# ucuapps/OpenGlue

Hardware: NVIDIA H100
Metric: image-pairs/sec at N=M=2048, d=256, 9 GNN layers, 100 Sinkhorn iters (higher is better)
Workload: dtype fp16x3 (fp16 hi/lo operands with power-of-two tensor scales, 3 products, fp32 accumulate)

## Files before the change

openglue_b200/csrc/sinkhorn.cuh:

```cuda
#pragma once
#include "common.cuh"
#include "tc_common.cuh"
#include <math_constants.h>
#include <algorithm>

namespace og {

struct SinkArgs {
  static constexpr bool kBackward = false;
  const float* S; int64_t lds, strideS;
  const float* dustbin;
  int B, n, m, iters;
  float reg;
  float norm, log_a_last, log_b_last;
  float* scores;
  float* u;
  float* partial;
  unsigned int* barrier;
  int SP, rows_per_strip, mpad;
  int rows_smem;
  float* vglob;
  float* hist_u;
  float* hist_v;
};

constexpr int SINK_WARPS = 8;
constexpr int64_t SINK_BARRIER_BYTES = 256 * 128;
constexpr int SINK_MAX_COLS = 8192;
constexpr int SINK_MAX_STRIPS = 32;
constexpr float LOG2E_F = 1.4426950408889634f;

__device__ __forceinline__ void grid_barrier(unsigned int* counter, unsigned int target) {
  __syncthreads();
  if (threadIdx.x == 0) {
    __threadfence();
    atomicAdd(counter, 1u);
    unsigned int seen;
    do {
      asm volatile("ld.acquire.gpu.global.u32 %0, [%1];" : "=r"(seen) : "l"(counter) : "memory");
    } while (seen < target);
    __threadfence();
  }
  __syncthreads();
}

typedef unsigned long long f32x2;
__device__ __forceinline__ f32x2 pk2(float x, float y) { f32x2 r; asm("mov.b64 %0, {%1, %2};" : "=l"(r) : "f"(x), "f"(y)); return r; }
__device__ __forceinline__ void upk2(f32x2 v, float& x, float& y) { asm("mov.b64 {%0, %1}, %2;" : "=f"(x), "=f"(y) : "l"(v)); }
#define OG_F32X2_OP(name, expr)                                        \
  __device__ __forceinline__ f32x2 name(f32x2 a, f32x2 b) {            \
    float ax, ay, bx, by; upk2(a, ax, ay); upk2(b, bx, by);            \
    auto op = [](float u, float v) { return expr; };                   \
    return pk2(op(ax, bx), op(ay, by));                                \
  }
OG_F32X2_OP(add2, __fadd_rn(u, v))
OG_F32X2_OP(sub2, __fsub_rn(u, v))
OG_F32X2_OP(mul2, __fmul_rn(u, v))
#undef OG_F32X2_OP
__device__ __forceinline__ f32x2 fma2(f32x2 a, f32x2 b, f32x2 c) {
  float ax, ay, bx, by, cx, cy; upk2(a, ax, ay); upk2(b, bx, by); upk2(c, cx, cy);
  return pk2(__fmaf_rn(ax, bx, cx), __fmaf_rn(ay, by, cy));
}

template <int V, int W>
struct SinkStrip {
  static constexpr int C = 128 * V, MC = W * C, G = SINK_WARPS / W;
  int b, strip, tid, lane, grp, sub, c0, r0, r1;
  template <class Args>
  __device__ __forceinline__ explicit SinkStrip(const Args& a) {
    b = blockIdx.x / a.SP; strip = blockIdx.x % a.SP;
    tid = threadIdx.x; lane = tid & 31;
    grp = (tid >> 5) / W; sub = (tid >> 5) % W;
    c0 = sub * C;
    r0 = strip * a.rows_per_strip;
    r1 = min(r0 + a.rows_per_strip, a.n + 1);
  }
};

template <int V, int W, int SLOTS, bool EVICT_FIRST, class Args>
struct SinkRowRing {
  static constexpr int C = 128 * V, G = SINK_WARPS / W;
  float* slot;
  uint64_t* bar;
  const Args& a;
  const float* seg;
  int first, end_real, c0, lane;
  uint32_t bytes, consumed;
  bool full;
  float dz;
  uint64_t policy;

  __device__ __forceinline__ SinkRowRing(const Args& args, const SinkStrip<V, W>& s, float* ring, uint64_t* bars) : a(args) {
    const int warp = s.grp * W + s.sub;
    slot = ring + warp * SLOTS * C;
    bar = bars + warp * SLOTS;
    seg = a.S + (int64_t)s.b * a.strideS + s.c0;
    first = s.r0 + s.grp;
    end_real = min(s.r1, a.n);
    c0 = s.c0; lane = s.lane;
    const int seg_cols = min(a.m, c0 + C) - c0;
    bytes = seg_cols > 0 ? (uint32_t)(((seg_cols + 3) / 4) * 16) : 0u;
    full = seg_cols == C;
    consumed = 0;
    dz = (a.reg == 1.0f) ? __ldg(a.dustbin) : __fdiv_rn(__ldg(a.dustbin), a.reg);
    if (lane == 0) {
      for (int sl = 0; sl < SLOTS; ++sl) tc::mbar_init(&bar[sl], 1);
      tc::fence_barrier_init();
    }
    if (EVICT_FIRST) asm volatile("createpolicy.fractional.L2::evict_first.b64 %0, 1.0;" : "=l"(policy));
  }

  __device__ __forceinline__ void copy(uint32_t sl, int row) {
    tc::mbar_arrive_expect_tx(&bar[sl], bytes);
    const float* src = seg + (int64_t)row * a.lds;
    if (EVICT_FIRST)
      asm volatile("cp.async.bulk.shared::cluster.global.mbarrier::complete_tx::bytes.L2::cache_hint [%0], [%1], %2, [%3], %4;"
                   ::"r"(tc::smem_u32(slot + sl * C)), "l"(src), "r"(bytes), "r"(tc::smem_u32(&bar[sl])), "l"(policy) : "memory");
    else
      asm volatile("cp.async.bulk.shared::cluster.global.mbarrier::complete_tx::bytes [%0], [%1], %2, [%3];"
                   ::"r"(tc::smem_u32(slot + sl * C)), "l"(src), "r"(bytes), "r"(tc::smem_u32(&bar[sl])) : "memory");
  }

  __device__ __forceinline__ void prime() {
    if (lane == 0 && bytes) {
      for (int sl = 0; sl < SLOTS; ++sl) {
        const int row = first + sl * G;
        if (row < end_real) copy((consumed + sl) % SLOTS, row);
      }
    }
  }

  __device__ __forceinline__ void take(int row, float4 (&z)[V]) {
    if (row >= a.n) {
#pragma unroll
      for (int k = 0; k < V; ++k) z[k] = make_float4(dz, dz, dz, dz);
      return;
    }
    if (!bytes) {
#pragma unroll
      for (int k = 0; k < V; ++k) z[k] = make_float4(0.f, 0.f, 0.f, 0.f);
      return;
    }
    const uint32_t sl = consumed % SLOTS, ph = (consumed / SLOTS) & 1;
    while (!tc::mbar_try_wait(&bar[sl], ph)) {}
    const float4* src = reinterpret_cast<const float4*>(slot + sl * C);
    if (full) {
#pragma unroll
      for (int k = 0; k < V; ++k) z[k] = src[lane + 32 * k];
    } else {
#pragma unroll
      for (int k = 0; k < V; ++k) {
        const int idx = lane + 32 * k;
        const int c = c0 + 4 * idx;
        const int m = a.m;
        float4 q = (c < m) ? src[idx] : make_float4(0.f, 0.f, 0.f, 0.f);
        if (c < m && c + 3 >= m) {
          if (c + 1 >= m) q.y = 0.f;
          if (c + 2 >= m) q.z = 0.f;
          q.w = 0.f;
        }
        z[k] = q;
      }
    }
    ++consumed;
    __syncwarp();
    const int nxt = row + SLOTS * G;
    if (lane == 0 && nxt < end_real) copy(sl, nxt);
    if (a.reg != 1.0f) {
      const float reg = a.reg;
#pragma unroll
      for (int k = 0; k < V; ++k) {
        z[k].x = __fdiv_rn(z[k].x, reg); z[k].y = __fdiv_rn(z[k].y, reg);
        z[k].z = __fdiv_rn(z[k].z, reg); z[k].w = __fdiv_rn(z[k].w, reg);
      }
    }
  }
};

template <int V, int W, class X>
__device__ __forceinline__ const X* sink_row_exchange(X* xr, X mine, const SinkStrip<V, W>& s, uint32_t& rowpar) {
  X* x = xr + (rowpar * SinkStrip<V, W>::G + s.grp) * W;
  if (s.lane == 0) x[s.sub] = mine;
  asm volatile("bar.sync %0, %1;" ::"r"(1 + s.grp), "n"(W * 32) : "memory");
  rowpar ^= 1u;
  return x;
}

template <int V, int W, class Args, class Store>
__device__ __forceinline__ void sink_strip_sums(const Args& a, const SinkStrip<V, W>& s, float* red, const float4 (&cacc)[V],
                                                float cacc_m, Store store) {
  const int m = a.m;
  float* myred = red + s.grp * a.mpad;
#pragma unroll
  for (int q = 0; q < V; ++q) {
    const int c = s.c0 + 4 * (s.lane + 32 * q);
    if (c < m) *reinterpret_cast<float4*>(myred + c) = cacc[q];
  }
  __syncthreads();
  if (s.sub == 0 && s.lane == 0) myred[m] = cacc_m;
  __syncthreads();
  for (int j = s.tid; j <= m; j += blockDim.x) {
    float sum = 0.f;
#pragma unroll
    for (int w = 0; w < SinkStrip<V, W>::G; ++w) sum += red[w * a.mpad + j];
    store(j, sum);
  }
}

template <int V, int W, class Args, class Update>
__device__ __forceinline__ void sink_column_reduce(const Args& a, const SinkStrip<V, W>& s, float* red, const float4 (&cacc)[V],
                                                   float cacc_m, int k, Update update) {
  const int m = a.m;
  const int64_t buf = (int64_t)(k & 1) * a.B * a.SP + (int64_t)s.b * a.SP;
  float* part = a.partial + (buf + s.strip) * a.mpad;
  sink_strip_sums(a, s, red, cacc, cacc_m, [&](int j, float sum) { part[j] = sum; });
  grid_barrier(a.barrier + 32 * s.b, (unsigned int)(k + 1) * (unsigned int)a.SP);
  const float* pb = a.partial + buf * a.mpad;
  for (int j4 = s.tid; 4 * j4 <= m; j4 += blockDim.x) {
    float4 c = make_float4(0.f, 0.f, 0.f, 0.f);
#pragma unroll 8
    for (int sp = 0; sp < a.SP; ++sp) {
      const float4 q = __ldcg(reinterpret_cast<const float4*>(pb + (int64_t)sp * a.mpad) + j4);
      c.x += q.x; c.y += q.y; c.z += q.z; c.w += q.w;
    }
    const float cc[4] = {c.x, c.y, c.z, c.w};
#pragma unroll
    for (int e = 0; e < 4; ++e) {
      const int j = 4 * j4 + e;
      if (j < m) update(j, cc[e]);
      else if (j == m) update(SinkStrip<V, W>::MC, cc[e]);
    }
  }
  __syncthreads();
}

template <int V, int W>
__device__ __forceinline__ void sink_fwd_row(const SinkArgs& a, const SinkStrip<V, W>& s, const float4 (&q)[V], const float* v_s,
                                             float v_m, float dz, float a_reg, float a_last, float2* xr, uint32_t& rowpar, int row,
                                             int it, f32x2 (&cacc)[2 * V], float& cacc_m) {
  const int n = a.n, c0 = s.c0, lane = s.lane, sub = s.sub;
  const f32x2 log2e2 = pk2(LOG2E_F, LOG2E_F);
  f32x2 z[2 * V];
#pragma unroll
  for (int k = 0; k < V; ++k) { z[2 * k] = pk2(q[k].x, q[k].y); z[2 * k + 1] = pk2(q[k].z, q[k].w); }
  const float t_m = dz + v_m;
  float mx = (sub == 0) ? t_m : -CUDART_INF_F;
#pragma unroll
  for (int k = 0; k < V; ++k) {
    const ulonglong2 vv = *reinterpret_cast<const ulonglong2*>(v_s + c0 + 4 * (lane + 32 * k));
    z[2 * k] = add2(z[2 * k], vv.x); z[2 * k + 1] = add2(z[2 * k + 1], vv.y);
    float x0, x1, x2, x3; upk2(z[2 * k], x0, x1); upk2(z[2 * k + 1], x2, x3);
    mx = fmaxf(mx, fmaxf(fmaxf(x0, x1), fmaxf(x2, x3)));
  }
  mx = warp_max(mx);
  const float mxs = (mx == -CUDART_INF_F) ? 0.f : mx;
  const f32x2 mxs2 = pk2(mxs, mxs);
  f32x2 sum2a = 0ull, sum2b = 0ull;
#pragma unroll
  for (int k = 0; k < 2 * V; ++k) {
    float x, y; upk2(mul2(sub2(z[k], mxs2), log2e2), x, y);
    z[k] = pk2(ex2_approx(x), ex2_approx(y));
    if (k & 1) sum2b = add2(sum2b, z[k]); else sum2a = add2(sum2a, z[k]);
  }
  float sa, sb; upk2(add2(sum2a, sum2b), sa, sb);
  const float e_m = (sub == 0) ? ex2_approx((t_m - mxs) * LOG2E_F) : 0.f;
  float s_i = warp_sum(sa + sb) + e_m;
  float mxg = mx, f_w = 1.f;
  if (W > 1) {
    const float2* x = sink_row_exchange(xr, make_float2(mx, s_i), s, rowpar);
    float2 p[W];
#pragma unroll
    for (int w2 = 0; w2 < W; ++w2) { p[w2] = x[w2]; mxg = fmaxf(mxg, p[w2].x); }
    s_i = 0.f;
#pragma unroll
    for (int w2 = 0; w2 < W; ++w2) s_i = fmaf(p[w2].y, ex2_approx((p[w2].x - mxg) * LOG2E_F), s_i);
    f_w = ex2_approx((mx - mxg) * LOG2E_F);
  }
  const float w_i = __fdiv_rn((row < n) ? a_reg : a_last, s_i) * f_w;
  if ((it == a.iters - 1 || a.hist_u) && sub == 0 && lane == 0) {
    const float u_i = ((row < n) ? a.norm : a.log_a_last) - (mxg + logf(s_i));
    if (it == a.iters - 1) a.u[(int64_t)s.b * (n + 1) + row] = u_i;
    if (a.hist_u) a.hist_u[((int64_t)s.b * a.iters + it) * (n + 1) + row] = u_i;
  }
  const f32x2 w2 = pk2(w_i, w_i);
#pragma unroll
  for (int k = 0; k < 2 * V; ++k) cacc[k] = fma2(z[k], w2, cacc[k]);
  cacc_m = fmaf(e_m, w_i, cacc_m);
}

template <int V, int W>
__device__ __forceinline__ void sink_fwd_score_row(const SinkArgs& a, const SinkStrip<V, W>& s, const float4 (&z)[V], const float* v_s,
                                                   float v_m, float dz, int row) {
  const int n = a.n, m = a.m, c0 = s.c0, lane = s.lane;
  float u_i = 0.f;
  if (a.iters > 0) {
    if (lane == 0) u_i = __ldcg(a.u + (int64_t)s.b * (n + 1) + row);
    u_i = __shfl_sync(0xffffffffu, u_i, 0);
  }
  float* out = a.scores + ((int64_t)s.b * (n + 1) + row) * (m + 1);
#pragma unroll
  for (int k = 0; k < V; ++k) {
    const int c = c0 + 4 * (lane + 32 * k);
    if (c < m) {
      const float4 vv = *reinterpret_cast<const float4*>(v_s + c);
      if (c + 0 < m) out[c + 0] = (z[k].x + u_i) + vv.x - a.norm;
      if (c + 1 < m) out[c + 1] = (z[k].y + u_i) + vv.y - a.norm;
      if (c + 2 < m) out[c + 2] = (z[k].z + u_i) + vv.z - a.norm;
      if (c + 3 < m) out[c + 3] = (z[k].w + u_i) + vv.w - a.norm;
    }
  }
  if (s.sub == 0 && lane == 0) out[m] = (dz + u_i) + v_m - a.norm;
}

template <int V, int W, int SLOTS>
__global__ void __launch_bounds__(SINK_WARPS * 32, (V <= 8) ? 2 : 1) sinkhorn_kernel(SinkArgs a) {
  extern __shared__ __align__(128) float og_sink_smem[];
  using Strip = SinkStrip<V, W>;
  constexpr int C = Strip::C, MC = Strip::MC, G = Strip::G;
  float* v_s = og_sink_smem;
  float* red = og_sink_smem + MC + 4;
  float* ring = red + G * a.mpad;
  uint64_t* bars = reinterpret_cast<uint64_t*>(ring + SINK_WARPS * SLOTS * C);
  float2* xr = reinterpret_cast<float2*>(bars + SINK_WARPS * SLOTS);
  const Strip s(a);
  const int m = a.m;
  const float a_reg = expf(a.norm), a_last = expf(a.log_a_last);
  SinkRowRing<V, W, SLOTS, true, SinkArgs> rows(a, s, ring, bars);
  const float dz = rows.dz;

  for (int j = s.tid; j < MC; j += blockDim.x) v_s[j] = (j < m) ? 0.f : -CUDART_INF_F;
  if (s.tid == 0) v_s[MC] = 0.f;
  __syncthreads();

  rows.prime();
  uint32_t rowpar = 0;
  for (int it = 0; it < a.iters; ++it) {
    f32x2 cacc[2 * V];
#pragma unroll
    for (int k = 0; k < 2 * V; ++k) cacc[k] = 0ull;
    float cacc_m = 0.f;
    const float v_m = v_s[MC];

    for (int row = s.r0 + s.grp; row < s.r1; row += G) {
      float4 q[V];
      rows.take(row, q);
      sink_fwd_row(a, s, q, v_s, v_m, dz, a_reg, a_last, xr, rowpar, row, it, cacc, cacc_m);
    }
    rows.prime();
    float4 c4[V];
#pragma unroll
    for (int k = 0; k < V; ++k) { upk2(cacc[2 * k], c4[k].x, c4[k].y); upk2(cacc[2 * k + 1], c4[k].z, c4[k].w); }
    sink_column_reduce(a, s, red, c4, cacc_m, it, [&](int j, float c) {
      v_s[j] = ((j < MC) ? a.norm : a.log_b_last) + v_s[j] - logf(c);
    });
    if (a.hist_v && s.strip == 0) {
      float* hv = a.hist_v + ((int64_t)s.b * (a.iters + 1) + it + 1) * (m + 1);
      for (int j = s.tid; j <= m; j += blockDim.x) hv[j] = (j < m) ? v_s[j] : v_s[MC];
    }
  }

  const float v_m = v_s[MC];
  for (int row = s.r0 + s.grp; row < s.r1; row += G) {
    float4 z[V];
    rows.take(row, z);
    sink_fwd_score_row(a, s, z, v_s, v_m, dz, row);
  }
}

__device__ __forceinline__ void sink_put(uint64_t* p, float x, uint32_t tag) {
  asm volatile("st.relaxed.gpu.global.b64 [%0], %1;" ::"l"(p), "l"(((uint64_t)tag << 32) | __float_as_uint(x)) : "memory");
}
__device__ __forceinline__ uint64_t sink_get(const uint64_t* p) {
  uint64_t w;
  asm volatile("ld.relaxed.gpu.global.b64 %0, [%1];" : "=l"(w) : "l"(p) : "memory");
  return w;
}
constexpr int SINK_POLL = 16;
template <int N, class At>
__device__ __forceinline__ void sink_take(float (&x)[N], At at, uint32_t tag) {
  uint64_t w[N];
#pragma unroll
  for (int u = 0; u < N; ++u) { const uint64_t* p = at(u); w[u] = p ? sink_get(p) : (uint64_t)tag << 32; }
  for (;;) {
    bool ready = true;
#pragma unroll
    for (int u = 0; u < N; ++u) ready &= (uint32_t)(w[u] >> 32) == tag;
    if (ready) break;
#pragma unroll
    for (int u = 0; u < N; ++u)
      if ((uint32_t)(w[u] >> 32) != tag) w[u] = sink_get(at(u));
  }
#pragma unroll
  for (int u = 0; u < N; ++u) x[u] = __uint_as_float((uint32_t)w[u]);
}

template <int V, int W, int RR>
__global__ void __launch_bounds__(SINK_WARPS * 32, 1) sinkhorn_resident_kernel(SinkArgs a) {
  extern __shared__ __align__(128) float og_sink_smem[];
  using Strip = SinkStrip<V, W>;
  constexpr int C = Strip::C, MC = Strip::MC, G = Strip::G, NT = SINK_WARPS * 32;
  float* v_s = og_sink_smem;
  float* red = v_s + MC + 4;
  float* ring = red;
  float* gsum = red + max(G * a.mpad, SINK_WARPS * C);
  float4* held = reinterpret_cast<float4*>(gsum + NT);
  uint64_t* bars = reinterpret_cast<uint64_t*>(held + (size_t)SINK_WARPS * a.rows_smem * (C / 4));
  float2* xr = reinterpret_cast<float2*>(bars + SINK_WARPS);
  const Strip s(a);
  const int m = a.m, lane = s.lane;
  const float a_reg = expf(a.norm), a_last = expf(a.log_a_last);
  SinkRowRing<V, W, 1, true, SinkArgs> rows(a, s, ring, bars);
  const float dz = rows.dz;
  float4* mine = held + (size_t)(s.grp * W + s.sub) * a.rows_smem * (C / 4);
  uint64_t* vg = reinterpret_cast<uint64_t*>(a.vglob) + (int64_t)s.b * a.mpad;

  for (int j = s.tid; j < MC; j += blockDim.x) v_s[j] = (j < m) ? 0.f : -CUDART_INF_F;
  if (s.tid == 0) v_s[MC] = 0.f;
  __syncthreads();

  rows.prime();
  uint32_t rowpar = 0;
  float4 zr[RR][V];
  for (int it = 0; it <= a.iters; ++it) {
    const bool last = it == a.iters;
    f32x2 cacc[2 * V];
#pragma unroll
    for (int k = 0; k < 2 * V; ++k) cacc[k] = 0ull;
    float cacc_m = 0.f;
    const float v_m = v_s[MC];
    auto visit = [&](int row, const float4 (&q)[V]) {
      if (last) sink_fwd_score_row(a, s, q, v_s, v_m, dz, row);
      else sink_fwd_row(a, s, q, v_s, v_m, dz, a_reg, a_last, xr, rowpar, row, it, cacc, cacc_m);
    };
#pragma unroll
    for (int k = 0; k < RR; ++k) {
      const int row = s.r0 + s.grp + k * G;
      if (row < s.r1) {
        if (it == 0) rows.take(row, zr[k]);
        visit(row, zr[k]);
      }
    }
    float4* h = mine;
    for (int row = s.r0 + s.grp + RR * G; row < s.r1; row += G, h += C / 4) {
      float4 q[V];
      if (it == 0) {
        rows.take(row, q);
#pragma unroll
        for (int k = 0; k < V; ++k) h[lane + 32 * k] = q[k];
      } else {
#pragma unroll
        for (int k = 0; k < V; ++k) q[k] = h[lane + 32 * k];
      }
      visit(row, q);
    }
    if (last) break;

    float4 c4[V];
#pragma unroll
    for (int k = 0; k < V; ++k) { upk2(cacc[2 * k], c4[k].x, c4[k].y); upk2(cacc[2 * k + 1], c4[k].z, c4[k].w); }
    if (it == 0) __syncthreads();
    const uint32_t tag = it + 1;
    uint64_t* pt = reinterpret_cast<uint64_t*>(a.partial) + (int64_t)s.b * a.SP * a.mpad;
    sink_strip_sums(a, s, red, c4, cacc_m, [&](int j, float sum) { sink_put(pt + (int64_t)s.strip * a.mpad + j, sum, tag); });
    const int S = cdiv(m + 1, a.SP), lo = s.strip * S, NG = S >= NT ? 1 : NT / S;
    auto publish = [&](int j, float c) {
      sink_put(vg + j, ((j < m) ? a.norm + v_s[j] : a.log_b_last + v_s[MC]) - logf(c), tag);
    };
    for (int i = s.tid; i < S * NG; i += NT) {
      const int j = lo + i % S;
      float sum = 0.f;
      if (j <= m) {
        for (int sp0 = i / S; sp0 < a.SP; sp0 += SINK_POLL * NG) {
          float x[SINK_POLL];
          sink_take<SINK_POLL>(x, [&](int u) { const int sp = sp0 + u * NG; return sp < a.SP ? pt + (int64_t)sp * a.mpad + j : nullptr; }, tag);
#pragma unroll
          for (int u = 0; u < SINK_POLL; ++u) sum += x[u];
        }
      }
      if (NG > 1) gsum[i] = sum;
      else if (j <= m) publish(j, sum);
    }
    if (NG > 1) {
      __syncthreads();
      for (int i = s.tid; i < S && lo + i <= m; i += NT) {
        float sum = gsum[i];
        for (int g = 1; g < NG; ++g) sum += gsum[g * S + i];
        publish(lo + i, sum);
      }
    }
    for (int j0 = s.tid; j0 <= m; j0 += SINK_POLL * NT) {
      float x[SINK_POLL];
      sink_take<SINK_POLL>(x, [&](int u) { const int j = j0 + u * NT; return j <= m ? vg + j : nullptr; }, tag);
#pragma unroll
      for (int u = 0; u < SINK_POLL; ++u) {
        const int j = j0 + u * NT;
        if (j <= m) v_s[(j < m) ? j : MC] = x[u];
      }
    }
    __syncthreads();
  }
}

struct SinkPlan { int V, W, slots, occ, SP, rows_per_strip, mpad, pairs_per_launch; size_t smem; bool resident; int rows_reg, rows_smem; };

constexpr size_t sinkhorn_smem(bool backward, int V, int W, int slots, int mpad) {
  const int C = 128 * V, G = SINK_WARPS / W, vecs = backward ? 3 : 1;
  const size_t xbytes = backward ? sizeof(float) : sizeof(float2);
  return ((size_t)vecs * (W * C + 4) + (size_t)G * mpad + (size_t)SINK_WARPS * slots * C) * sizeof(float) +
         (size_t)SINK_WARPS * slots * sizeof(uint64_t) + (size_t)2 * G * W * xbytes + 128;
}

inline int sinkhorn_plan(bool backward, int B, int n, int m, SinkPlan* p) {
  const char* who = backward ? "sinkhorn_bwd" : "sinkhorn";
  if (m <= 512)                { p->V = 4;  p->W = 1; p->slots = 2; }
  else if (m <= 1024)          { p->V = 4;  p->W = 2; p->slots = 2; }
  else if (m <= 2048)          { p->V = 8;  p->W = 2; p->slots = 2; }
  else if (m <= 4096)          { p->V = 16; p->W = 2; p->slots = backward ? 1 : 2; }
  else if (m <= SINK_MAX_COLS) { p->V = 16; p->W = 4; p->slots = 1; }
  else return fail(OG_EUNSUPPORTED, "%s: m = %d > %d columns not supported (swap the images)", who, m, SINK_MAX_COLS);
  p->mpad = (int)align_up(m + 1, 4);
  p->smem = sinkhorn_smem(backward, p->V, p->W, p->slots, p->mpad);
  p->occ = (p->V <= 8 && 2 * (p->smem + 1024) <= OG_SMEM_OPTIN_MAX) ? 2 : 1;
  const int sms = device_info().ok ? device_info().sm_count : 132;
  const int ctas = sms * p->occ;
  p->pairs_per_launch = std::min(B < ctas ? B : ctas, (int)(SINK_BARRIER_BYTES / 128));
  int sp = std::min(ctas / p->pairs_per_launch, SINK_MAX_STRIPS);
  const int max_sp = cdiv(n + 1, SINK_WARPS / p->W);
  if (sp > max_sp) sp = max_sp;
  if (sp < 1) sp = 1;
  p->SP = sp;
  p->rows_per_strip = cdiv(n + 1, sp);
  return OG_OK;
}

constexpr size_t sinkhorn_resident_smem(int V, int W, int mpad, int rows_smem) {
  const int C = 128 * V, G = SINK_WARPS / W;
  return ((size_t)(W * C + 4) + (size_t)std::max(G * mpad, SINK_WARPS * C) + 4 * SINK_WARPS * 32 +
          (size_t)SINK_WARPS * rows_smem * C) * sizeof(float) +
         SINK_WARPS * sizeof(uint64_t) + (size_t)2 * G * W * sizeof(float2) + 128;
}

inline bool sinkhorn_resident_plan(int B, int n, int m, SinkPlan* p) {
  if (m > 2048 || sinkhorn_plan(false, B, n, m, p) != OG_OK) return false;
  const int G = SINK_WARPS / p->W, rr = 24 / p->V, C = 128 * p->V;
  const int sms = device_info().ok ? device_info().sm_count : 132;
  const int rs_max = (int)((OG_SMEM_OPTIN_MAX - sinkhorn_resident_smem(p->V, p->W, p->mpad, 0)) / (SINK_WARPS * C * sizeof(float)));
  const int sp_min = cdiv(n + 1, G * (rr + rs_max));
  if (2 * sp_min > sms) return false;
  const int rounds = cdiv(B, std::min(B, sms / sp_min));
  p->pairs_per_launch = cdiv(B, rounds);
  const int sp = std::min(sms / p->pairs_per_launch, cdiv(n + 1, G));
  p->rows_per_strip = cdiv(n + 1, sp);
  p->SP = cdiv(n + 1, p->rows_per_strip);
  const int rows_per_warp = cdiv(p->rows_per_strip, G);
  const double resident_us = rounds * (3.8 + rows_per_warp * (0.4 + 0.0625 * p->V));
  const double streaming_us = 4.0 * B * (n + 1) * (m + 1) / 2.7e6;
  if (rounds > 1 && resident_us >= streaming_us) return false;
  p->rows_reg = rr;
  p->rows_smem = std::max(0, rows_per_warp - rr);
  p->smem = sinkhorn_resident_smem(p->V, p->W, p->mpad, p->rows_smem);
  p->slots = 1; p->occ = 1; p->resident = true;
  return true;
}

inline int& sink_resident_mode() {
  static int v = [] { const char* e = getenv("OG_SINK_RESIDENT"); return e ? (atoi(e) != 0) : 1; }();
  return v;
}

inline int sinkhorn_check_rows(const char* who, const float* S, int64_t lds, int64_t strideS, int m) {
  if (lds % 4 != 0 || lds < m || !aligned16(S) || strideS % 4 != 0)
    return fail(OG_EINVAL, "%s: S rows must be 16-byte aligned (lds %% 4 == 0, lds >= m)", who);
  return OG_OK;
}

struct SinkConsts { float norm, log_a_last, log_b_last; };
inline SinkConsts sinkhorn_consts(int n, int m) {
  const float norm = -logf((float)(n + m));
  return {norm, norm + (float)log((double)m),
          norm + (float)log((double)n)};
}

template <auto Kernel, int V, int W, int SLOTS, class Args>
inline int sinkhorn_coop_launch(const Args& a, const SinkPlan& p, cudaStream_t stream) {
  constexpr size_t smem_max = sinkhorn_smem(Args::kBackward, V, W, SLOTS, 128 * V * W + 4);
  static_assert(smem_max <= OG_SMEM_OPTIN_MAX, "Sinkhorn kernel: shared memory beyond what one block may opt in to");
  if (const int rc = smem_opt_in<Kernel>((int)smem_max)) return rc;
  return launch(Args::kBackward ? "sinkhorn_bwd_kernel" : "sinkhorn_kernel", Kernel, LaunchAttr::cooperative, dim3(a.B * a.SP),
                dim3(SINK_WARPS * 32), p.smem, stream, a);
}

template <class Launch>
inline int sinkhorn_for_each_launch(const SinkPlan& p, int B, unsigned int* barrier, cudaStream_t stream, Launch&& launch) {
  for (int b0 = 0; b0 < B; b0 += p.pairs_per_launch) {
    const int nb = std::min(p.pairs_per_launch, B - b0);
    OG_CUDA(cudaMemsetAsync(barrier, 0, (size_t)nb * 128, stream));
    if (const int rc = launch(b0, nb)) return rc;
  }
  return OG_OK;
}

inline int64_t sinkhorn_workspace_bytes(int B, int n, int m) {
  SinkPlan p, r;
  if (sinkhorn_plan(false, B, n, m, &p) != OG_OK) return -1;
  int64_t rows = 2LL * B * SINK_MAX_STRIPS;
  if (sinkhorn_resident_plan(B, n, m, &r)) rows = std::max<int64_t>(rows, 2LL * (r.SP + 1) * r.pairs_per_launch);
  return SINK_BARRIER_BYTES + align_up((int64_t)B * (n + 1) * 4, 256) + align_up(rows * p.mpad * 4, 256);
}

template <int V, int W>
inline int sinkhorn_resident_launch(const SinkArgs& a, const SinkPlan& p, cudaStream_t stream) {
  constexpr auto kernel = sinkhorn_resident_kernel<V, W, 24 / V>;
  if (const int rc = smem_opt_in<kernel>((int)OG_SMEM_OPTIN_MAX)) return rc;
  return launch("sinkhorn_resident_kernel", kernel, LaunchAttr::cooperative, dim3(a.B * a.SP), dim3(SINK_WARPS * 32), p.smem,
                stream, a);
}

inline int sinkhorn_launch(const float* S, int64_t lds, int64_t strideS, const float* dustbin, int B, int n, int m,
                           int iters, float reg, float* scores, void* ws, int64_t ws_bytes, cudaStream_t stream,
                           float* hist_u = nullptr, float* hist_v = nullptr) {
  SinkPlan p;
  const bool resident = !hist_u && !hist_v && sink_resident_mode() && sinkhorn_resident_plan(B, n, m, &p);
  if (!resident) {
    if (const int rc = sinkhorn_plan(false, B, n, m, &p)) return rc;
    p.resident = false;
  }
  if (ws_bytes < sinkhorn_workspace_bytes(B, n, m)) return fail(OG_EWORKSPACE, "sinkhorn: workspace too small");
  if (const int rc = sinkhorn_check_rows("sinkhorn", S, lds, strideS, m)) return rc;
  char* w = static_cast<char*>(ws);
  unsigned int* barrier = reinterpret_cast<unsigned int*>(w); w += SINK_BARRIER_BYTES;
  float* u = reinterpret_cast<float*>(w); w += align_up((int64_t)B * (n + 1) * 4, 256);
  float* partial = reinterpret_cast<float*>(w);
  const SinkConsts k = sinkhorn_consts(n, m);
  if (hist_v) OG_CUDA(cudaMemsetAsync(hist_v, 0, (size_t)B * (iters + 1) * (m + 1) * sizeof(float), stream));
  return sinkhorn_for_each_launch(p, B, barrier, stream, [&](int b0, int nb) {
    SinkArgs a;
    a.S = S + (int64_t)b0 * strideS; a.lds = lds; a.strideS = strideS; a.dustbin = dustbin;
    a.B = nb; a.n = n; a.m = m; a.iters = iters; a.reg = reg;
    a.norm = k.norm; a.log_a_last = k.log_a_last; a.log_b_last = k.log_b_last;
    a.scores = scores + (int64_t)b0 * (n + 1) * (m + 1);
    a.u = u; a.partial = partial; a.barrier = barrier;
    a.SP = p.SP; a.rows_per_strip = p.rows_per_strip; a.mpad = p.mpad;
    a.rows_smem = p.resident ? p.rows_smem : 0;
    a.vglob = partial + 2LL * p.pairs_per_launch * p.SP * p.mpad;
    if (p.resident) OG_CUDA(cudaMemsetAsync(partial, 0, 8LL * (p.SP + 1) * p.pairs_per_launch * p.mpad, stream));
    a.hist_u = hist_u ? hist_u + (int64_t)b0 * iters * (n + 1) : nullptr;
    a.hist_v = hist_v ? hist_v + (int64_t)b0 * (iters + 1) * (m + 1) : nullptr;
    if (p.resident) {
      if (p.W == 1) return sinkhorn_resident_launch<4, 1>(a, p, stream);
      return p.V == 4 ? sinkhorn_resident_launch<4, 2>(a, p, stream) : sinkhorn_resident_launch<8, 2>(a, p, stream);
    }
    if (p.V == 4 && p.W == 1) return sinkhorn_coop_launch<sinkhorn_kernel<4, 1, 2>, 4, 1, 2>(a, p, stream);
    if (p.V == 4)             return sinkhorn_coop_launch<sinkhorn_kernel<4, 2, 2>, 4, 2, 2>(a, p, stream);
    if (p.V == 8)             return sinkhorn_coop_launch<sinkhorn_kernel<8, 2, 2>, 8, 2, 2>(a, p, stream);
    if (p.W == 2)             return sinkhorn_coop_launch<sinkhorn_kernel<16, 2, 2>, 16, 2, 2>(a, p, stream);
    return sinkhorn_coop_launch<sinkhorn_kernel<16, 4, 1>, 16, 4, 1>(a, p, stream);
  });
}

}
```

Baseline: 480.5.

## Process two Sinkhorn rows per step and fold strip sums in resident kernel

Result: faster. 497.7, median of 6 (+3.6%).

```diff
diff --git a/openglue_b200/csrc/sinkhorn.cuh b/openglue_b200/csrc/sinkhorn.cuh
--- a/openglue_b200/csrc/sinkhorn.cuh
+++ b/openglue_b200/csrc/sinkhorn.cuh
@@ -3,6 +3,7 @@
 #include "tc_common.cuh"
 #include <math_constants.h>
 #include <algorithm>
+#include <type_traits>
 
 namespace og {
 
@@ -234,58 +235,98 @@
   __syncthreads();
 }
 
-template <int V, int W>
-__device__ __forceinline__ void sink_fwd_row(const SinkArgs& a, const SinkStrip<V, W>& s, const float4 (&q)[V], const float* v_s,
-                                             float v_m, float dz, float a_reg, float a_last, float2* xr, uint32_t& rowpar, int row,
-                                             int it, f32x2 (&cacc)[2 * V], float& cacc_m) {
+template <int NR> using SinkRowStat = std::conditional_t<NR == 1, float2, float4>;
+
+template <int V, int W, int NR>
+__device__ __forceinline__ void sink_fwd_rows(const SinkArgs& a, const SinkStrip<V, W>& s, const float4 (*q)[V], const float* v_s,
+                                              float v_m, float dz, float a_reg, float a_last, SinkRowStat<NR>* xr, uint32_t& rowpar,
+                                              int row0, int it, f32x2 (&cacc)[2 * V], float& cacc_m) {
+  static_assert(NR == 1 || NR == 2, "one or two rows at a time");
   const int n = a.n, c0 = s.c0, lane = s.lane, sub = s.sub;
   const f32x2 log2e2 = pk2(LOG2E_F, LOG2E_F);
-  f32x2 z[2 * V];
-#pragma unroll
-  for (int k = 0; k < V; ++k) { z[2 * k] = pk2(q[k].x, q[k].y); z[2 * k + 1] = pk2(q[k].z, q[k].w); }
+  f32x2 z[NR][2 * V];
+#pragma unroll
+  for (int r = 0; r < NR; ++r)
+#pragma unroll
+    for (int k = 0; k < V; ++k) { z[r][2 * k] = pk2(q[r][k].x, q[r][k].y); z[r][2 * k + 1] = pk2(q[r][k].z, q[r][k].w); }
   const float t_m = dz + v_m;
-  float mx = (sub == 0) ? t_m : -CUDART_INF_F;
+  float mx[NR];
+#pragma unroll
+  for (int r = 0; r < NR; ++r) mx[r] = (sub == 0) ? t_m : -CUDART_INF_F;
 #pragma unroll
   for (int k = 0; k < V; ++k) {
     const ulonglong2 vv = *reinterpret_cast<const ulonglong2*>(v_s + c0 + 4 * (lane + 32 * k));
-    z[2 * k] = add2(z[2 * k], vv.x); z[2 * k + 1] = add2(z[2 * k + 1], vv.y);
-    float x0, x1, x2, x3; upk2(z[2 * k], x0, x1); upk2(z[2 * k + 1], x2, x3);
-    mx = fmaxf(mx, fmaxf(fmaxf(x0, x1), fmaxf(x2, x3)));
-  }
-  mx = warp_max(mx);
-  const float mxs = (mx == -CUDART_INF_F) ? 0.f : mx;
-  const f32x2 mxs2 = pk2(mxs, mxs);
-  f32x2 sum2a = 0ull, sum2b = 0ull;
-#pragma unroll
-  for (int k = 0; k < 2 * V; ++k) {
-    float x, y; upk2(mul2(sub2(z[k], mxs2), log2e2), x, y);
-    z[k] = pk2(ex2_approx(x), ex2_approx(y));
-    if (k & 1) sum2b = add2(sum2b, z[k]); else sum2a = add2(sum2a, z[k]);
-  }
-  float sa, sb; upk2(add2(sum2a, sum2b), sa, sb);
-  const float e_m = (sub == 0) ? ex2_approx((t_m - mxs) * LOG2E_F) : 0.f;
-  float s_i = warp_sum(sa + sb) + e_m;
-  float mxg = mx, f_w = 1.f;
+#pragma unroll
+    for (int r = 0; r < NR; ++r) {
+      z[r][2 * k] = add2(z[r][2 * k], vv.x); z[r][2 * k + 1] = add2(z[r][2 * k + 1], vv.y);
+      float x0, x1, x2, x3; upk2(z[r][2 * k], x0, x1); upk2(z[r][2 * k + 1], x2, x3);
+      mx[r] = fmaxf(mx[r], fmaxf(fmaxf(x0, x1), fmaxf(x2, x3)));
+    }
+  }
+#pragma unroll
+  for (int r = 0; r < NR; ++r) mx[r] = warp_max(mx[r]);
+  float s_i[NR], e_m[NR];
+#pragma unroll
+  for (int r = 0; r < NR; ++r) {
+    const float mxs = (mx[r] == -CUDART_INF_F) ? 0.f : mx[r];
+    const f32x2 mxs2 = pk2(mxs, mxs);
+    f32x2 sum2a = 0ull, sum2b = 0ull;
+#pragma unroll
+    for (int k = 0; k < 2 * V; ++k) {
+      float x, y; upk2(mul2(sub2(z[r][k], mxs2), log2e2), x, y);
+      z[r][k] = pk2(ex2_approx(x), ex2_approx(y));
+      if (k & 1) sum2b = add2(sum2b, z[r][k]); else sum2a = add2(sum2a, z[r][k]);
+    }
+    float sa, sb; upk2(add2(sum2a, sum2b), sa, sb);
+    s_i[r] = sa + sb;
+    e_m[r] = (sub == 0) ? ex2_approx((t_m - mxs) * LOG2E_F) : 0.f;
+  }
+#pragma unroll
+  for (int r = 0; r < NR; ++r) s_i[r] = warp_sum(s_i[r]) + e_m[r];
+  float mxg[NR], f_w[NR];
+#pragma unroll
+  for (int r = 0; r < NR; ++r) { mxg[r] = mx[r]; f_w[r] = 1.f; }
   if (W > 1) {
-    const float2* x = sink_row_exchange(xr, make_float2(mx, s_i), s, rowpar);
-    float2 p[W];
-#pragma unroll
-    for (int w2 = 0; w2 < W; ++w2) { p[w2] = x[w2]; mxg = fmaxf(mxg, p[w2].x); }
-    s_i = 0.f;
-#pragma unroll
-    for (int w2 = 0; w2 < W; ++w2) s_i = fmaf(p[w2].y, ex2_approx((p[w2].x - mxg) * LOG2E_F), s_i);
-    f_w = ex2_approx((mx - mxg) * LOG2E_F);
-  }
-  const float w_i = __fdiv_rn((row < n) ? a_reg : a_last, s_i) * f_w;
+    SinkRowStat<NR> mine;
+    if constexpr (NR == 1) mine = make_float2(mx[0], s_i[0]);
+    else mine = make_float4(mx[0], s_i[0], mx[1], s_i[1]);
+    const SinkRowStat<NR>* x = sink_row_exchange(xr, mine, s, rowpar);
+    float pm[NR][W], ps[NR][W];
+#pragma unroll
+    for (int w2 = 0; w2 < W; ++w2) {
+      const SinkRowStat<NR> p = x[w2];
+      pm[0][w2] = p.x; ps[0][w2] = p.y;
+      if constexpr (NR == 2) { pm[1][w2] = p.z; ps[1][w2] = p.w; }
+    }
+#pragma unroll
+    for (int r = 0; r < NR; ++r) {
+#pragma unroll
+      for (int w2 = 0; w2 < W; ++w2) mxg[r] = fmaxf(mxg[r], pm[r][w2]);
+      s_i[r] = 0.f;
+#pragma unroll
+      for (int w2 = 0; w2 < W; ++w2) s_i[r] = fmaf(ps[r][w2], ex2_approx((pm[r][w2] - mxg[r]) * LOG2E_F), s_i[r]);
+      f_w[r] = ex2_approx((mx[r] - mxg[r]) * LOG2E_F);
+    }
+  }
+  float w_i[NR];
+#pragma unroll
+  for (int r = 0; r < NR; ++r) w_i[r] = __fdiv_rn((row0 + r * SinkStrip<V, W>::G < n) ? a_reg : a_last, s_i[r]) * f_w[r];
   if ((it == a.iters - 1 || a.hist_u) && sub == 0 && lane == 0) {
-    const float u_i = ((row < n) ? a.norm : a.log_a_last) - (mxg + logf(s_i));
-    if (it == a.iters - 1) a.u[(int64_t)s.b * (n + 1) + row] = u_i;
-    if (a.hist_u) a.hist_u[((int64_t)s.b * a.iters + it) * (n + 1) + row] = u_i;
-  }
-  const f32x2 w2 = pk2(w_i, w_i);
-#pragma unroll
-  for (int k = 0; k < 2 * V; ++k) cacc[k] = fma2(z[k], w2, cacc[k]);
-  cacc_m = fmaf(e_m, w_i, cacc_m);
+#pragma unroll
+    for (int r = 0; r < NR; ++r) {
+      const int row = row0 + r * SinkStrip<V, W>::G;
+      const float u_i = ((row < n) ? a.norm : a.log_a_last) - (mxg[r] + logf(s_i[r]));
+      if (it == a.iters - 1) a.u[(int64_t)s.b * (n + 1) + row] = u_i;
+      if (a.hist_u) a.hist_u[((int64_t)s.b * a.iters + it) * (n + 1) + row] = u_i;
+    }
+  }
+#pragma unroll
+  for (int r = 0; r < NR; ++r) {
+    const f32x2 w2 = pk2(w_i[r], w_i[r]);
+#pragma unroll
+    for (int k = 0; k < 2 * V; ++k) cacc[k] = fma2(z[r][k], w2, cacc[k]);
+    cacc_m = fmaf(e_m[r], w_i[r], cacc_m);
+  }
 }
 
 template <int V, int W>
@@ -344,7 +385,7 @@
     for (int row = s.r0 + s.grp; row < s.r1; row += G) {
       float4 q[V];
       rows.take(row, q);
-      sink_fwd_row(a, s, q, v_s, v_m, dz, a_reg, a_last, xr, rowpar, row, it, cacc, cacc_m);
+      sink_fwd_rows<V, W, 1>(a, s, &q, v_s, v_m, dz, a_reg, a_last, xr, rowpar, row, it, cacc, cacc_m);
     }
     rows.prime();
     float4 c4[V];
@@ -394,24 +435,61 @@
   for (int u = 0; u < N; ++u) x[u] = __uint_as_float((uint32_t)w[u]);
 }
 
+template <int V, int W, class Args, class Store>
+__device__ __forceinline__ void sink_strip_sums_folded(const Args& a, const SinkStrip<V, W>& s, float* red, float* redm,
+                                                       const float4 (&cacc)[V], float cacc_m, Store store) {
+  constexpr int H = SinkStrip<V, W>::G / 2;
+  const int m = a.m;
+  float4* fold = reinterpret_cast<float4*>(red + (s.grp % H) * a.mpad);
+  if (s.grp >= H) {
+#pragma unroll
+    for (int q = 0; q < V; ++q) {
+      const int c = s.c0 + 4 * (s.lane + 32 * q);
+      if (c < m) fold[c / 4] = cacc[q];
+    }
+  }
+  if (s.sub == 0 && s.lane == 0) redm[s.grp] = cacc_m;
+  __syncthreads();
+  if (s.grp < H) {
+#pragma unroll
+    for (int q = 0; q < V; ++q) {
+      const int c = s.c0 + 4 * (s.lane + 32 * q);
+      if (c < m) {
+        const float4 o = fold[c / 4];
+        fold[c / 4] = make_float4(cacc[q].x + o.x, cacc[q].y + o.y, cacc[q].z + o.z, cacc[q].w + o.w);
+      }
+    }
+  }
+  __syncthreads();
+  for (int j = s.tid; j <= m; j += blockDim.x) {
+    float sum = 0.f;
+#pragma unroll
+    for (int h = 0; h < H; ++h) sum += (j < m) ? red[h * a.mpad + j] : redm[h] + redm[h + H];
+    store(j, sum);
+  }
+}
+
 template <int V, int W, int RR>
 __global__ void __launch_bounds__(SINK_WARPS * 32, 1) sinkhorn_resident_kernel(SinkArgs a) {
+  static_assert(RR % 2 == 0, "the register rows go two at a time");
   extern __shared__ __align__(128) float og_sink_smem[];
   using Strip = SinkStrip<V, W>;
-  constexpr int C = Strip::C, MC = Strip::MC, G = Strip::G, NT = SINK_WARPS * 32;
+  constexpr int C = Strip::C, MC = Strip::MC, G = Strip::G, NT = SINK_WARPS * 32, HS = SINK_WARPS * (C / 4);
+  const int slots = max(a.rows_smem, 1);
   float* v_s = og_sink_smem;
   float* red = v_s + MC + 4;
-  float* ring = red;
-  float* gsum = red + max(G * a.mpad, SINK_WARPS * C);
+  float* gsum = red + G / 2 * a.mpad;
   float4* held = reinterpret_cast<float4*>(gsum + NT);
-  uint64_t* bars = reinterpret_cast<uint64_t*>(held + (size_t)SINK_WARPS * a.rows_smem * (C / 4));
+  uint64_t* bars = reinterpret_cast<uint64_t*>(held + (size_t)slots * HS);
   float2* xr = reinterpret_cast<float2*>(bars + SINK_WARPS);
+  float4* xr2 = reinterpret_cast<float4*>(xr + 2 * G * W);
+  float* redm = reinterpret_cast<float*>(xr2 + 2 * G * W);
   const Strip s(a);
-  const int m = a.m, lane = s.lane;
+  const int m = a.m, lane = s.lane, row0 = s.r0 + s.grp;
   const float a_reg = expf(a.norm), a_last = expf(a.log_a_last);
-  SinkRowRing<V, W, 1, true, SinkArgs> rows(a, s, ring, bars);
+  float4* mine = held + (s.grp * W + s.sub) * (C / 4);
+  SinkRowRing<V, W, 1, true, SinkArgs> rows(a, s, reinterpret_cast<float*>(held + (size_t)(slots - 1) * HS), bars);
   const float dz = rows.dz;
-  float4* mine = held + (size_t)(s.grp * W + s.sub) * a.rows_smem * (C / 4);
   uint64_t* vg = reinterpret_cast<uint64_t*>(a.vglob) + (int64_t)s.b * a.mpad;
 
   for (int j = s.tid; j < MC; j += blockDim.x) v_s[j] = (j < m) ? 0.f : -CUDART_INF_F;
@@ -420,7 +498,7 @@
 
   rows.prime();
   uint32_t rowpar = 0;
-  float4 zr[RR][V];
+  float4 zr[RR / 2][2][V];
   for (int it = 0; it <= a.iters; ++it) {
     const bool last = it == a.iters;
     f32x2 cacc[2 * V];
@@ -428,40 +506,70 @@
     for (int k = 0; k < 2 * V; ++k) cacc[k] = 0ull;
     float cacc_m = 0.f;
     const float v_m = v_s[MC];
-    auto visit = [&](int row, const float4 (&q)[V]) {
-      if (last) sink_fwd_score_row(a, s, q, v_s, v_m, dz, row);
-      else sink_fwd_row(a, s, q, v_s, v_m, dz, a_reg, a_last, xr, rowpar, row, it, cacc, cacc_m);
+    auto one = [&](int row, const float4 (*q)[V]) {
+      sink_fwd_rows<V, W, 1>(a, s, q, v_s, v_m, dz, a_reg, a_last, xr, rowpar, row, it, cacc, cacc_m);
     };
-#pragma unroll
-    for (int k = 0; k < RR; ++k) {
-      const int row = s.r0 + s.grp + k * G;
+    if (it == 0 || last) {
+      auto visit = [&](int row, const float4 (&q)[V]) {
+        if (last) sink_fwd_score_row(a, s, q, v_s, v_m, dz, row);
+        else one(row, &q);
+      };
+#pragma unroll
+      for (int k = 0; k < RR; ++k) {
+        const int row = row0 + k * G;
+        if (row < s.r1) {
+          if (it == 0) rows.take(row, zr[k / 2][k % 2]);
+          visit(row, zr[k / 2][k % 2]);
+        }
+      }
+      float4* h = mine;
+      for (int row = row0 + RR * G; row < s.r1; row += G, h += HS) {
+        float4 q[V];
+        if (it == 0) {
+          rows.take(row, q);
+#pragma unroll
+          for (int k = 0; k < V; ++k) h[lane + 32 * k] = q[k];
+        } else {
+#pragma unroll
+          for (int k = 0; k < V; ++k) q[k] = h[lane + 32 * k];
+        }
+        visit(row, q);
+      }
+      if (last) break;
+    } else {
+      auto two = [&](int row, const float4 (*q)[V]) {
+        sink_fwd_rows<V, W, 2>(a, s, q, v_s, v_m, dz, a_reg, a_last, xr2, rowpar, row, it, cacc, cacc_m);
+      };
+#pragma unroll
+      for (int k = 0; k < RR; k += 2) {
+        const int row = row0 + k * G;
+        if (row + G < s.r1) two(row, zr[k / 2]);
+        else if (row < s.r1) one(row, zr[k / 2]);
+      }
+      const float4* h = mine;
+      int row = row0 + RR * G;
+      for (; row + G < s.r1; row += 2 * G, h += 2 * HS) {
+        float4 q[2][V];
+#pragma unroll
+        for (int r = 0; r < 2; ++r)
+#pragma unroll
+          for (int k = 0; k < V; ++k) q[r][k] = h[r * HS + lane + 32 * k];
+        two(row, q);
+      }
       if (row < s.r1) {
-        if (it == 0) rows.take(row, zr[k]);
-        visit(row, zr[k]);
-      }
-    }
-    float4* h = mine;
-    for (int row = s.r0 + s.grp + RR * G; row < s.r1; row += G, h += C / 4) {
-      float4 q[V];
-      if (it == 0) {
-        rows.take(row, q);
-#pragma unroll
-        for (int k = 0; k < V; ++k) h[lane + 32 * k] = q[k];
-      } else {
-#pragma unroll
-        for (int k = 0; k < V; ++k) q[k] = h[lane + 32 * k];
-      }
-      visit(row, q);
-    }
-    if (last) break;
+        float4 q[1][V];
+#pragma unroll
+        for (int k = 0; k < V; ++k) q[0][k] = h[lane + 32 * k];
+        one(row, q);
+      }
+    }
 
     float4 c4[V];
 #pragma unroll
     for (int k = 0; k < V; ++k) { upk2(cacc[2 * k], c4[k].x, c4[k].y); upk2(cacc[2 * k + 1], c4[k].z, c4[k].w); }
-    if (it == 0) __syncthreads();
     const uint32_t tag = it + 1;
     uint64_t* pt = reinterpret_cast<uint64_t*>(a.partial) + (int64_t)s.b * a.SP * a.mpad;
-    sink_strip_sums(a, s, red, c4, cacc_m, [&](int j, float sum) { sink_put(pt + (int64_t)s.strip * a.mpad + j, sum, tag); });
+    sink_strip_sums_folded(a, s, red, redm, c4, cacc_m, [&](int j, float sum) { sink_put(pt + (int64_t)s.strip * a.mpad + j, sum, tag); });
     const int S = cdiv(m + 1, a.SP), lo = s.strip * S, NG = S >= NT ? 1 : NT / S;
     auto publish = [&](int j, float c) {
       sink_put(vg + j, ((j < m) ? a.norm + v_s[j] : a.log_b_last + v_s[MC]) - logf(c), tag);
@@ -535,16 +643,16 @@
 
 constexpr size_t sinkhorn_resident_smem(int V, int W, int mpad, int rows_smem) {
   const int C = 128 * V, G = SINK_WARPS / W;
-  return ((size_t)(W * C + 4) + (size_t)std::max(G * mpad, SINK_WARPS * C) + 4 * SINK_WARPS * 32 +
-          (size_t)SINK_WARPS * rows_smem * C) * sizeof(float) +
-         SINK_WARPS * sizeof(uint64_t) + (size_t)2 * G * W * sizeof(float2) + 128;
+  return ((size_t)(W * C + 4) + (size_t)G / 2 * mpad + 4 * SINK_WARPS * 32 + (size_t)SINK_WARPS * std::max(rows_smem, 1) * C) *
+             sizeof(float) +
+         SINK_WARPS * sizeof(uint64_t) + (size_t)2 * G * W * (sizeof(float2) + sizeof(float4)) + G * sizeof(float) + 128;
 }
 
 inline bool sinkhorn_resident_plan(int B, int n, int m, SinkPlan* p) {
   if (m > 2048 || sinkhorn_plan(false, B, n, m, p) != OG_OK) return false;
-  const int G = SINK_WARPS / p->W, rr = 24 / p->V, C = 128 * p->V;
+  const int G = SINK_WARPS / p->W, rr = 16 / p->V, C = 128 * p->V;
   const int sms = device_info().ok ? device_info().sm_count : 132;
-  const int rs_max = (int)((OG_SMEM_OPTIN_MAX - sinkhorn_resident_smem(p->V, p->W, p->mpad, 0)) / (SINK_WARPS * C * sizeof(float)));
+  const int rs_max = 1 + (int)((OG_SMEM_OPTIN_MAX - sinkhorn_resident_smem(p->V, p->W, p->mpad, 1)) / (SINK_WARPS * C * sizeof(float)));
   const int sp_min = cdiv(n + 1, G * (rr + rs_max));
   if (2 * sp_min > sms) return false;
   const int rounds = cdiv(B, std::min(B, sms / sp_min));
@@ -610,7 +718,7 @@
 
 template <int V, int W>
 inline int sinkhorn_resident_launch(const SinkArgs& a, const SinkPlan& p, cudaStream_t stream) {
-  constexpr auto kernel = sinkhorn_resident_kernel<V, W, 24 / V>;
+  constexpr auto kernel = sinkhorn_resident_kernel<V, W, 16 / V>;
   if (const int rc = smem_opt_in<kernel>((int)OG_SMEM_OPTIN_MAX)) return rc;
   return launch("sinkhorn_resident_kernel", kernel, LaunchAttr::cooperative, dim3(a.B * a.SP), dim3(SINK_WARPS * 32), p.smem,
                 stream, a);
```
